# RobustFieldAutonomyLab/Distributional_RL_Navigation

Hardware: AMD Instinct MI355X
Metric: env steps/sec (whole node) at 65 536 envs; IQN grad-steps/sec (higher is better)
Workload: dtype f32; 1 GPU; 65536 envs/GPU + IQN training (act K=32, 8 quantiles, replay 100000, batch 256, 1 grad step(s) every 4 vector steps); envs_per_gpu=65536, n_cores=8, n_obstacles=10, precision=f64, learner=independent, ranks_per_gpu=1, act_variant=2, taus=per_env, resets=under_next_act, launches_per_grad_step=1, ablation=False

## Files before the change

distributional_rl_navigation_amd/csrc/mn_capi.hip:

```cpp
#include <math.h>
#include <stdio.h>
#include <stdlib.h>
#include <string.h>

#include <string>
#include <vector>

#include "mn_internal.h"
#include "mn_render_font.h"

struct mn_handle {
    MnArrays A;
    MnDev P;
    mn_params params;
    std::vector<void *> allocs;
    std::string err;
    int step_parity = 0;
    int last_parity = 0;
    uint32_t *seeds_dev = nullptr;
    uint32_t *mask_count = nullptr;
    int32_t *list_scratch = nullptr;
    double *peek_scratch = nullptr;
    double *obs64_buf = nullptr, *rew64_buf = nullptr;
    double *traj_trace = nullptr;
    int32_t traj_trace_steps = 0, traj_trace_sub = 0;
    int device = -1;
    std::vector<hipEvent_t> ev;
    int prof_max = 0, prof_n = 0;
    std::vector<hipEvent_t> ev_reset;
    int prof_reset_n = 0;
    hipStream_t side = nullptr;
    hipEvent_t ev_stepped = nullptr, ev_reset_end = nullptr;
    uint32_t *ready = nullptr;
    uint32_t tick = 0;
    bool reset_pending = false;
    volatile uint32_t *seen_host = nullptr;
    uint32_t *seen_dev = nullptr, *peak_dev = nullptr;
    int32_t under_act_max = MN_RESET_UNDER_ACT_MAX_DEFAULT;
// ... 140 lines not shown
    h->params = p;
    return MN_OK;
}

template <typename T>
static int dev_alloc(mn_handle *h, T **out, size_t count, bool zero = true) {
    void *p = nullptr;
    hipError_t e = hipMalloc(&p, count * sizeof(T));
    if (e != hipSuccess) { h->err = std::string("hipMalloc failed: ") + hipGetErrorString(e); return MN_ERR_ALLOC; }
    if (zero) { e = hipMemset(p, 0, count * sizeof(T)); if (e != hipSuccess) { h->err = hipGetErrorString(e); return MN_ERR_HIP; } }
    h->allocs.push_back(p);
    *out = (T *)p;
    return MN_OK;
}

extern "C" int mn_destroy(mn_handle *h) {
    if (!h) return MN_ERR_INVALID;
    int cur = -1;
    const bool moved = hipGetDevice(&cur) == hipSuccess && h->device >= 0 && cur != h->device;
    if (moved) (void)hipSetDevice(h->device);
    if (h->reset_owed) { const hipStream_t s = h->owed_stream; settle_owed(h, s); (void)hipStreamSynchronize(s); }
    for (hipEvent_t e : h->ev) (void)hipEventDestroy(e);
    for (hipEvent_t e : h->ev_reset) (void)hipEventDestroy(e);
    if (h->side) { (void)hipStreamSynchronize(h->side); (void)hipStreamDestroy(h->side); }
    if (h->ev_stepped) (void)hipEventDestroy(h->ev_stepped);
    if (h->ev_reset_end) (void)hipEventDestroy(h->ev_reset_end);
    if (h->seen_host) (void)hipHostFree((void *)h->seen_host);
    for (void *p : h->allocs) (void)hipFree(p);
    if (moved) (void)hipSetDevice(cur);
    delete h;
// ... 40 lines not shown
    {
        std::vector<double> v(np);
        for (size_t i = 0; i < np; ++i) v[i] = 5.0;
        (void)hipMemcpy(A.start_x, v.data(), np * 8, hipMemcpyHostToDevice);
        (void)hipMemcpy(A.start_y, v.data(), np * 8, hipMemcpyHostToDevice);
        for (size_t i = 0; i < np; ++i) v[i] = 45.0;
        (void)hipMemcpy(A.goal_x, v.data(), np * 8, hipMemcpyHostToDevice);
        (void)hipMemcpy(A.goal_y, v.data(), np * 8, hipMemcpyHostToDevice);
        std::vector<uint32_t> s(np);
        for (size_t i = 0; i < np; ++i) s[i] = (uint32_t)i;
        rc = mn_seed(h, s.data(), nullptr);
        if (rc) { g_create_err = h->err; mn_destroy(h); return rc; }
        hipError_t e = hipDeviceSynchronize();
        if (e != hipSuccess) { g_create_err = hipGetErrorString(e); mn_destroy(h); return MN_ERR_HIP; }
    }
    *out = h;
    return MN_OK;
}

extern "C" const char *mn_last_error(const mn_handle *h) { return h ? h->err.c_str() : g_create_err.c_str(); }
extern "C" int32_t mn_num_envs(const mn_handle *h) { return h ? h->A.n : 0; }

extern "C" int mn_set_params(mn_handle *h, const mn_params *p) {
    if (!h || !p) return MN_ERR_INVALID;
    if (p->precision != h->params.precision) return fail(h, MN_ERR_INVALID, "precision is fixed at mn_create");
    if (h->reset_owed) MN_ON_DEVICE(h);
    return derive(h, *p);
}

extern "C" int mn_get_params(const mn_handle *h, mn_params *p) {
// ... 395 lines not shown

extern "C" int mn_set_reset_owed_max_rows(mn_handle *h, int32_t owed_max_rows) {
    if (!h) return MN_ERR_INVALID;
    h->owed_max_rows = owed_max_rows;
    return MN_OK;
}

extern "C" int32_t mn_reset_is_owed(const mn_handle *h) { return h && h->reset_owed ? 1 : 0; }

bool mn_owed_reset_take(mn_handle *h, hipStream_t s, MnOwedReset *out) {
    if (!h || !h->reset_owed) return false;
    int cur = -1;
    if (hipGetDevice(&cur) != hipSuccess || cur != h->device) return false;
    if (s != h->owed_stream) (void)hipStreamSynchronize(h->owed_stream);
    const bool prof = h->prof_reset_n < h->prof_max;
    *out = MnOwedReset{&h->A, &h->P, h->params.precision, h->A.queue_count + h->last_parity * MN_QWORDS, h->A.queue, h->owed_obs, h->peak_dev, h->seen_dev,
                       mn_prep_reset_blocks(*h->seen_host, h->A.n), prof ? h->ev_reset[2 * h->prof_reset_n] : nullptr,
                       prof ? h->ev_reset[2 * h->prof_reset_n + 1] : nullptr};
    if (prof) h->prof_reset_n++;
    h->reset_owed = false;
    return true;
}
int mn_owed_reset_settle(mn_handle *h, hipStream_t s) {
    if (!h) return MN_OK;
    join_reset(h, s);
    return h->reset_owed ? fail(h, MN_ERR_INVALID, "the handle's owed reset lives on another HIP device") : MN_OK;
}

extern "C" int mn_set_reset_under_act_max(mn_handle *h, int32_t under_act_max, int64_t *last_seen) {
    if (!h) return MN_ERR_INVALID;
    h->under_act_max = under_act_max;
// ... 457 lines not shown
    int rc = range_ok(h, first, count);
    if (rc) return rc;
    if (count == 0) return MN_OK;
    if (!out) return MN_ERR_INVALID;
    if (!h->A.rew64) return fail(h, MN_ERR_INVALID, "float64 rewards are kept only with MN_PRECISION_F64 after mn_enable_obs64(h, 1)");
    MN_HIP(h, hipDeviceSynchronize());
    MN_HIP(h, hipMemcpy(out, h->A.rew64 + first, (size_t)count * 8, hipMemcpyDeviceToHost));
    return MN_OK;
}

extern "C" int mn_enable_obs64(mn_handle *h, int32_t on) {
    if (!h || on < 0 || on > 1) return MN_ERR_INVALID;
    MN_ON_DEVICE(h);
    if (h->params.precision != MN_PRECISION_F64) return fail(h, MN_ERR_INVALID, "float64 observation copies exist only with MN_PRECISION_F64");
    MN_HIP(h, hipDeviceSynchronize());
    if (!on) { h->A.obs64 = nullptr; h->A.rew64 = nullptr; return MN_OK; }
    if (!h->obs64_buf) {
        int rc = dev_alloc(h, &h->obs64_buf, (size_t)h->A.npad * MN_OBS_DIM);
        if (rc == MN_OK) rc = dev_alloc(h, &h->rew64_buf, (size_t)h->A.npad);
        if (rc) return rc;
    }
    h->A.obs64 = h->obs64_buf; h->A.rew64 = h->rew64_buf;
    return MN_OK;
}

extern "C" int mn_enable_trajectory(mn_handle *h, int32_t max_substeps) {
    if (!h || max_substeps < 1 || max_substeps > 1000) return MN_ERR_INVALID;
    MN_ON_DEVICE(h);
    if (h->params.precision != MN_PRECISION_F64) return fail(h, MN_ERR_INVALID, "sub-step trajectories are recorded only with MN_PRECISION_F64");
    if (h->A.traj && h->A.traj_n >= max_substeps) return MN_OK;
    MN_HIP(h, hipDeviceSynchronize());
    int rc = dev_alloc(h, &h->A.traj, (size_t)h->A.npad * max_substeps * 2);
    if (rc) return rc;
    h->A.traj_n = max_substeps;
    return MN_OK;
}

extern "C" int mn_get_trajectory(mn_handle *h, int32_t first, int32_t count, int32_t n_substeps, double *out) {
    int rc = range_ok(h, first, count);
    if (rc) return rc;
    if (count == 0) return MN_OK;
    if (!out || n_substeps < 1) return MN_ERR_INVALID;
    if (!h->A.traj || n_substeps > h->A.traj_n) return fail(h, MN_ERR_INVALID, "call mn_enable_trajectory(h, >= n_substeps) before stepping");
    MN_HIP(h, hipDeviceSynchronize());
    MN_HIP(h, hipMemcpy2D(out, (size_t)n_substeps * 16, h->A.traj + (size_t)first * h->A.traj_n * 2, (size_t)h->A.traj_n * 16,
                          (size_t)n_substeps * 16, count, hipMemcpyDeviceToHost));
    return MN_OK;
}

extern "C" int mn_peek_next_double(mn_handle *h, int32_t first, int32_t count, double *out) {
// ... 75 lines not shown
```

distributional_rl_navigation_amd/csrc/mn_internal.h:

```cpp
#pragma once
#include <hip/hip_runtime.h>
#include <stdint.h>

#include "marinenav_hip.h"

#define MN_WAVE 64
#define MN_PAD 256
#define MN_FIX_SCALE 16777216.0
#define MN_FIX_INV (1.0 / 16777216.0)
#define MN_TAB_ROWS (3 * MN_MAX_CORES + 3 * MN_MAX_OBS)

struct MnArrays {
    int32_t n, npad;
    double *x, *y, *theta, *speed, *vx, *vy;
    double *start_x, *start_y, *goal_x, *goal_y, *init_theta, *init_speed;
    int32_t *ep_t;
    int64_t *tot_t;
    int32_t *counts;
    double *cx, *cy, *cg;
    double *ox, *oy, *orad;
    int32_t *qcx, *qcy, *qox, *qoy;
    float *qcg, *qor;
    uint32_t *mt;
    int32_t *mt_pos;
// ... 99 lines not shown
int mn_iqn_rollout_image(mn_iqn_ctx *c, const float *const *weights, hipStream_t s, const uint32_t **image, uint32_t **words);
void mn_launch_dqn_pack(const float *const *weights, float *image_dev, hipStream_t s);
void mn_launch_rollout_dqn(const MnArrays &A, const MnDev &P, int precision, int n_steps, const float *image, float *obs_io, float *obs_trace,
                           float *reward_trace, uint8_t *done_trace, uint8_t *info_trace, int32_t *action_trace, float *q_trace, double *traj_trace, hipStream_t s);
void mn_launch_rollout_dqn_groups(const MnArrays &A, const MnDev &P, int precision, int n_steps, const float *images, int64_t image_stride, int n_groups,
                                  int rows_per_group, float *obs_io, float *obs_trace, float *reward_trace, uint8_t *done_trace, uint8_t *info_trace,
                                  int32_t *action_trace, float *q_trace, hipStream_t s);
void mn_launch_reset_under_act(const MnArrays &A, const MnDev &P, int precision, const uint32_t *count_dev, const int32_t *list_dev, float *obs,
                               uint32_t *ready, uint32_t tick, uint32_t *peak_dev, uint32_t *peak_host, hipStream_t s);
void mn_launch_reset(const MnArrays &A, const MnDev &P, int precision, const uint32_t *count_dev, uint32_t count_host,
                     const int32_t *list_dev, int mode, float *obs, hipStream_t s, uint32_t *peak_dev = nullptr, uint32_t *peak_host = nullptr, bool sharded = false);
#define MN_PREP_RESET_MIN_BLOCKS 256
#define MN_PREP_RESET_MAX_BLOCKS 8192
struct MnOwedReset {
    const MnArrays *A;
    const MnDev *P;
    int precision;
    const uint32_t *count_dev;
    const int32_t *list;
    float *obs;
    uint32_t *peak_dev, *peak_host;
    int blocks;
    hipEvent_t ev_begin, ev_end;
};
struct MnPrepLaunch {
    const float *const *weights;
    const float *consts;
    uint32_t *packed;
    bool pack;
    const uint64_t *rng_state;
// ... 33 lines not shown
```

distributional_rl_navigation_amd/csrc/mn_prep_reset.hip:

```cpp
#include <hip/hip_runtime.h>
#include <stdint.h>

#include "marinenav_hip.h"

#pragma clang fp contract(off)
#include "mn_reset_body.h"
#include "mn_done_queue.h"
#pragma clang fp contract(fast)

namespace {

#include "iqn_act_common.h"
#include "iqn_act_split.h"

constexpr int PR_PACK_BLOCKS = (sp::OFF_FB + MN_WAVE - 1) / MN_WAVE;

struct PrepArgs {
    IqnWeights w;
    const float *consts;
    uint32_t *packed;
    const uint64_t *rng_state;
    float *draws;
    int n;
    const float *cvar_row;
    float cvar;
    int pack_blocks;
    float eps;
    int32_t *actions;
    GreedyRows rows;
};

template <typename M, bool PARITY>
__global__ __launch_bounds__(MN_WAVE) void mn_prep_reset_kernel(MnArrays A, MnDev P, const uint32_t *__restrict__ count_dev, const int32_t *__restrict__ list,
                                                                float *__restrict__ obs_out, const MnSeen seen, int reset_blocks, PrepArgs a) {
    __shared__ MtLds S;
    __shared__ WorldLds W;
    if ((int)blockIdx.x < reset_blocks) {
        MnDoneQueue Q;
        const uint32_t count = Q.open(count_dev);
        mn_note_count(seen, count);
        for (uint32_t qi = blockIdx.x; qi < count; qi += (uint32_t)reset_blocks) mn_reset_env<M, PARITY>(A, P, S, W, Q.at(list, A.qcap, qi), 0, obs_out);
        return;
    }
    const int b = (int)blockIdx.x - reset_blocks;
    if (b < a.pack_blocks) {
        const int i = b * MN_WAVE + (int)threadIdx.x;
        if (i < sp::OFF_FB) a.packed[i] = sp::pack_word(a.w, a.consts, i);
        return;
    }
    if (a.rows.words) draw_block<true, MN_WAVE>(a.rng_state, a.draws, a.n, a.cvar_row, a.cvar, reset_blocks + a.pack_blocks, a.eps, a.actions, a.rows);
    else draw_block<false, MN_WAVE>(a.rng_state, a.draws, a.n, a.cvar_row, a.cvar, reset_blocks + a.pack_blocks);
}

}

int mn_prep_reset_blocks(uint32_t seen, int n) {
// ... 7 lines not shown
void mn_launch_prep_reset(const MnOwedReset &o, const MnPrepLaunch &p, hipStream_t s) {
    const MnSeen seen = {o.peak_dev, o.peak_host};
    PrepArgs a;
    const float *const *w = p.weights;
    a.w = {w[0], w[1], w[2], w[3], w[4], w[5], w[6], w[7], w[8], w[9], w[10], w[11], w[12], w[13]};
    a.consts = p.consts; a.packed = p.packed; a.rng_state = p.rng_state; a.draws = p.draws; a.n = p.n; a.cvar_row = p.cvar_row; a.cvar = p.cvar;
    a.pack_blocks = p.pack ? PR_PACK_BLOCKS : 0;
    a.eps = p.eps; a.actions = p.actions; a.rows = GreedyRows{p.rows_list, p.rows_words};
    const long items = ((long)p.n * (K_TAUS + 1) + 3) / 4;
    long draw = (items + MN_WAVE - 1) / MN_WAVE;
    if (draw > p.max_draw_blocks) draw = p.max_draw_blocks;
    if (draw < 1) draw = 1;
    const dim3 grid((unsigned)(o.blocks + a.pack_blocks + draw));
    if (o.ev_begin) (void)hipEventRecord(o.ev_begin, s);
    if (o.precision == MN_PRECISION_F64)
        hipLaunchKernelGGL((mn_prep_reset_kernel<double, true>), grid, dim3(MN_WAVE), 0, s, *o.A, *o.P, o.count_dev, o.list, o.obs, seen, o.blocks, a);
    else
        hipLaunchKernelGGL((mn_prep_reset_kernel<float, false>), grid, dim3(MN_WAVE), 0, s, *o.A, *o.P, o.count_dev, o.list, o.obs, seen, o.blocks, a);
    if (o.ev_end) (void)hipEventRecord(o.ev_end, s);
}
```

distributional_rl_navigation_amd/csrc/mn_reset.hip:

```cpp
#include "mn_reset_body.h"
#include "mn_done_queue.h"

#ifndef MN_RESET_MAX_BLOCKS
#define MN_RESET_MAX_BLOCKS 8192u
#endif

namespace {

template <typename M, bool PARITY>
__global__ __launch_bounds__(MN_WAVE) void mn_reset_kernel(MnArrays A, MnDev P, const uint32_t *__restrict__ count_dev,
                                                           uint32_t count_host, const int32_t *__restrict__ list, int mode,
                                                           float *__restrict__ obs_out, const MnSeen seen, int qcap) {
    __shared__ MtLds S;
    __shared__ WorldLds W;
    MnDoneQueue Q;
    const uint32_t count = qcap ? Q.open(count_dev) : (count_dev ? *count_dev : count_host);
    mn_note_count(seen, count);
    for (uint32_t qi = blockIdx.x; qi < count; qi += gridDim.x)
        mn_reset_env<M, PARITY>(A, P, S, W, qcap ? Q.at(list, qcap, qi) : (list ? list[qi] : (int)qi), mode, obs_out);
}

template <typename M, bool PARITY>
__global__ __launch_bounds__(MN_WAVE, 5) void mn_reset_under_act_kernel(MnArrays A, MnDev P, const uint32_t *__restrict__ count_dev,
                                                                        const int32_t *__restrict__ list, float *__restrict__ obs_out,
                                                                        uint32_t *__restrict__ ready, uint32_t tick, const MnSeen seen) {
    __shared__ MtCarryLds S;
    __shared__ WorldLds W;
    MnDoneQueue Q;
    const uint32_t count = Q.open(count_dev);
    mn_note_count(seen, count);
    for (uint32_t qi = blockIdx.x; qi < count; qi += gridDim.x)
        mn_reset_env<M, PARITY, MtInPlace>(A, P, S, W, Q.at(list, A.qcap, qi), 0, obs_out, ready, tick);
}

// ... 71 lines not shown
    while (__builtin_amdgcn_s_memrealtime() - t0 < 100ull * us) __builtin_amdgcn_s_sleep(64);
}
void mn_launch_sleep(uint32_t us, hipStream_t s) { hipLaunchKernelGGL(mn_sleep_kernel, dim3(1), dim3(MN_WAVE), 0, s, us); }

void mn_launch_seed(const MnArrays &A, const uint32_t *seeds_dev, hipStream_t s) {
    hipLaunchKernelGGL(mn_seed_kernel, dim3((A.n + 255) / 256), dim3(256), 0, s, A, seeds_dev);
}

void mn_launch_mask_to_queue(const MnArrays &A, const uint8_t *mask, uint32_t *count, int32_t *list, hipStream_t s) {
    hipLaunchKernelGGL(mn_mask_to_queue_kernel, dim3((A.n + 255) / 256), dim3(256), 0, s, A, mask, count, list);
}

void mn_launch_peek(const MnArrays &A, int first, int count, double *out_dev, hipStream_t s) {
    hipLaunchKernelGGL(mn_peek_kernel, dim3((count + 255) / 256), dim3(256), 0, s, A, first, count, out_dev);
}
```

distributional_rl_navigation_amd/csrc/mn_reset_body.h:

```cpp
#pragma once
#include "mn_device.h"

#ifdef MN_ABLATION
#define MN_RSKIP(bit) ((P.debug_skip & (bit)) != 0)
#else
#define MN_RSKIP(bit) false
#endif

#define MT_N 624
#define MT_M 397

__device__ __forceinline__ uint32_t mt_temper(uint32_t y) {
    y ^= (y >> 11);
    y ^= (y << 7) & 0x9d2c5680u;
    y ^= (y << 15) & 0xefc60000u;
    y ^= (y >> 18);
    return y;
}

__device__ __forceinline__ uint32_t mt_twist(uint32_t cur, uint32_t nxt, uint32_t far) {
    const uint32_t y = (cur & 0x80000000u) | (nxt & 0x7fffffffu);
    return far ^ (y >> 1) ^ ((y & 1u) ? 0x9908b0dfu : 0u);
}

struct MtLds {
    uint32_t key[MT_N];
    uint32_t carry[8];
};

__device__ __forceinline__ void mt_regenerate(MtLds &S, int lane) {
    for (int base = 0; base < MT_N - 1; base += MN_WAVE) {
        const int i = base + lane;
        uint32_t v = 0;
        const bool ok = i < MT_N - 1;
        if (ok) {
            const int j = i + MT_M < MT_N ? i + MT_M : i + MT_M - MT_N;
            v = mt_twist(S.key[i], S.key[i + 1], S.key[j]);
        }
        __syncthreads();
        if (ok) S.key[i] = v;
        __syncthreads();
    }
    if (lane == 0) S.key[MT_N - 1] = mt_twist(S.key[MT_N - 1], S.key[0], S.key[MT_M - 1]);
    __syncthreads();
}

struct MtCursor {
    int pos;
    int carry_n;
    bool regen;
};

__device__ __forceinline__ int mt_ensure(MtLds &S, MtCursor &c, int w, int lane) {
    int avail = c.carry_n + (MT_N - c.pos);
    if (avail < w) {
        const int rem = MT_N - c.pos;
        if (lane < rem) S.carry[c.carry_n + lane] = mt_temper(S.key[c.pos + lane]);
        __syncthreads();
        c.carry_n += rem;
        mt_regenerate(S, lane);
// ... 9 lines not shown
    return j < c.carry_n ? S.carry[j] : mt_temper(S.key[c.pos + j - c.carry_n]);
}

__device__ __forceinline__ double mt_double_at(const MtLds &S, const MtCursor &c, int j) {
    const uint32_t a = mt_word(S, c, j) >> 5, b = mt_word(S, c, j + 1) >> 6;
    return (a * 67108864.0 + b) / 9007199254740992.0;
}

__device__ __forceinline__ void mt_advance(MtCursor &c, int words) {
    c.pos += words - c.carry_n;
    c.carry_n = 0;
}

struct MtInLds {
    using Shared = MtLds;
    MtLds &S;
    MtCursor c;
    __device__ __forceinline__ MtInLds(MtLds &s) : S(s) {}
    __device__ __forceinline__ void load(const MnArrays &A, int e, int lane) {
        for (int j = lane; j < MT_N; j += MN_WAVE) S.key[j] = A.mt[(size_t)e * MT_N + j];
        c.pos = A.mt_pos[e];
        c.carry_n = 0;
        c.regen = false;
        __syncthreads();
    }
    __device__ __forceinline__ int ensure(int w, int lane) { return mt_ensure(S, c, w, lane); }
    template <int N>
    __device__ __forceinline__ void fetch(int j, double (&d)[N]) const {
#pragma unroll
        for (int q = 0; q < N; ++q) d[q] = mt_double_at(S, c, j + 2 * q);
    }
    __device__ __forceinline__ void advance(int words) { mt_advance(c, words); }
    __device__ __forceinline__ void store(const MnArrays &A, int e, int lane, bool skip) {
        if (c.regen && !skip) for (int j = lane; j < MT_N; j += MN_WAVE) A.mt[(size_t)e * MT_N + j] = S.key[j];
    }
};

struct MtCarryLds { uint32_t carry[8]; };
struct MtInPlace {
    using Shared = MtCarryLds;
    MtCarryLds &S;
    uint32_t *k;
    MtCursor c;
    __device__ __forceinline__ MtInPlace(MtCarryLds &s) : S(s), k(nullptr) {}
    static __device__ __forceinline__ uint32_t ld(const uint32_t *p) { return __hip_atomic_load(p, __ATOMIC_RELAXED, __HIP_MEMORY_SCOPE_AGENT); }
    static __device__ __forceinline__ void st(uint32_t *p, uint32_t v) { __hip_atomic_store(p, v, __ATOMIC_RELAXED, __HIP_MEMORY_SCOPE_AGENT); }
    __device__ __forceinline__ void load(const MnArrays &A, int e, int lane) {
        k = A.mt + (size_t)e * MT_N;
        c.pos = A.mt_pos[e];
        c.carry_n = 0;
        c.regen = false;
    }
    __device__ __forceinline__ void regenerate(int lane) {
        uint32_t a[4], b[4], u[4], v[4], f[4];
#pragma unroll
// ... 131 lines not shown
        if (d2 > t2 * (1.0 + 1.0e-11)) return true;
    } else {
        const double tr = 2 * P.core_r, tr2 = tr * tr;
        if (d2 < tr2 * (1.0 - 1.0e-11)) return true;
        if (d2 > tr2 * (1.0 + 1.0e-11)) {
            const double Gl = Gi > Gj ? Gi : Gj, Gs = Gi < Gj ? Gi : Gj;
            const double a = P.p * Gs, b = Gl * P.core_r + tr * a;
            const double lhs = a * a * d2, rhs = b * b;
            if (lhs < rhs * (1.0 - 1.0e-11)) return false;
            if (lhs > rhs * (1.0 + 1.0e-11)) return true;
        }
    }
    return cores_compatible_exact(P, sqrt(d2), gi, gj);
}

template <typename M, bool PARITY, typename RNG = MtInLds>
__device__ __forceinline__ void mn_reset_env(const MnArrays &A, const MnDev &P, typename RNG::Shared &S, WorldLds &W, int e, int mode,
                                             float *__restrict__ obs_out, uint32_t *__restrict__ ready = nullptr, uint32_t tick = 0u) {
    const int lane = threadIdx.x & (MN_WAVE - 1);
    const int np = A.npad;
    __syncthreads();
    int nc = 0, no = 0;
    double sx, sy, gx, gy, th0, sp0;

    if (mode == 0) {
        int want_c = P.num_cores, want_o = P.num_obs;
        double min_dis = P.min_start_goal_dis;
        if (P.n_stages > 0) {
            const int64_t tt = (int64_t)((double)A.tot_t[e] * P.timestep_scale);
            int cntle = 0;
            for (int i = 0; i < P.n_stages; ++i) cntle += (P.sched_t[i] - tt <= 0) ? 1 : 0;
            int idx = cntle - 1;
            if (idx < 0) idx += P.n_stages;
            want_c = P.sched_nc[idx]; want_o = P.sched_no[idx]; min_dis = P.sched_md[idx];
        }
        want_c = want_c > MN_MAX_CORES ? MN_MAX_CORES : want_c;
        want_o = want_o > MN_MAX_OBS ? MN_MAX_OBS : want_o;

        RNG rng(S);
        rng.load(A, e, lane);

        sx = A.start_x[e]; sy = A.start_y[e]; gx = A.goal_x[e]; gy = A.goal_y[e];
        if (P.reset_start_and_goal && !MN_RSKIP(32)) {
            int tried = 0;
            double best = 0.0;
            for (;;) {
                int nb = rng.ensure(8, lane);
                nb = nb < 500 - tried ? nb : 500 - tried;
                const bool mine = lane < nb;
                double s0 = 0, s1 = 0, g0 = 0, g1 = 0, d = -1.0;
                if (mine) {
                    double u[4];
                    rng.template fetch<4>(8 * lane, u);
                    s0 = P.sg_lo_x + P.sg_span_x * u[0];
                    s1 = P.sg_lo_y + P.sg_span_y * u[1];
                    g0 = P.sg_lo_x + P.sg_span_x * u[2];
                    g1 = P.sg_lo_y + P.sg_span_y * u[3];
// ... 13 lines not shown
                        if (od > bm || (od == bm && ol < bl)) { bm = od; bl = ol; }
                    }
                    pick = bm > best ? bl : -1;
                    used = nb; finished = (tried + nb) >= 500;
                }
                if (pick >= 0) {
                    best = bcast(d, pick);
                    sx = bcast(s0, pick); sy = bcast(s1, pick); gx = bcast(g0, pick); gy = bcast(g1, pick);
                }
                tried += used;
                rng.advance(8 * used);
                if (finished) break;
            }
        }

        if (want_c > 0 && !MN_RSKIP(64)) {
            int tried = 0;
            for (;;) {
                int nb = rng.ensure(8, lane);
                nb = nb < 500 - tried ? nb : 500 - tried;
                const bool mine = lane < nb;
                double x = 0, y = 0, g = 1.0;
                bool valid = false;
                if (mine) {
                    double u[4];
                    rng.template fetch<4>(8 * lane, u);
                    x = 0.0 + P.c_span_x * u[0];
                    y = 0.0 + P.c_span_y * u[1];
                    const bool clockwise = u[2] > P.binom_q;
                    const double v_edge = P.v_lo + P.v_span * u[3];
                    const double Gamma = P.two_pi_r * v_edge;
// ... 10 lines not shown
                    if (!m) break;
                    const int j = first_lane(m);
                    const double xj = bcast(x, j), yj = bcast(y, j), gj = bcast(g, j);
                    if (lane == j) { W.cx[nc] = x; W.cy[nc] = y; W.cg[nc] = g; valid = false; }
                    else if (valid && lane > j) valid = cores_compatible(P, xj, yj, gj, x, y, g);
                    ++nc;
                    if (nc == want_c) { used = j + 1; break; }
                }
                __syncthreads();
                tried += used;
                rng.advance(8 * used);
                if (nc == want_c || tried >= 500) break;
            }
        }

        if (want_o > 0 && !MN_RSKIP(128)) {
            int tried = 0;
            for (;;) {
                int nb = rng.ensure(6, lane);
                nb = nb < 500 - tried ? nb : 500 - tried;
                const bool mine = lane < nb;
                double x = 0, y = 0, r = 0;
                bool valid = false;
                if (mine) {
                    double u[3];
                    rng.template fetch<3>(6 * lane, u);
                    x = P.o_lo + P.o_span_x * u[0];
                    y = P.o_lo + P.o_span_y * u[1];
                    r = P.or_lo + P.or_span * u[2];
                    valid = !(x - r < 0.0 || x + r > P.width) && !(y - r < 0.0 || y + r > P.height) &&
                            !dist_lt((x - sx) * (x - sx) + (y - sy) * (y - sy), r + P.clear_r) &&
// ... 16 lines not shown
                    if (lane == j) { W.ox[no] = x; W.oy[no] = y; W.orad[no] = r; valid = false; }
                    else if (valid && lane > j) {
                        const double dx = xj - x, dy = yj - y;
                        valid = !dist_le(dx * dx + dy * dy, rj + r);
                    }
                    ++no;
                    if (no == want_o) { used = j + 1; break; }
                }
                __syncthreads();
                tried += used;
                rng.advance(6 * used);
                if (no == want_o || tried >= 500) break;
            }
        }

        if (P.random_reset_state) {
            rng.ensure(4, lane);
            double u[2];
            rng.template fetch<2>(0, u);
            th0 = 0.0 + (P.two_pi - 0.0) * u[0];
            sp0 = 0.0 + (P.max_speed - 0.0) * u[1];
            rng.advance(4);
        } else {
            th0 = P.init_theta; sp0 = P.init_speed;
        }

        __syncthreads();
        rng.store(A, e, lane, MN_RSKIP(512));
        if (lane < MN_MAX_CORES) {
            const bool v = lane < nc;
            A.cx[lane * np + e] = v ? W.cx[lane] : 0.0;
            A.cy[lane * np + e] = v ? W.cy[lane] : 0.0;
            A.cg[lane * np + e] = v ? W.cg[lane] : 0.0;
        }
        if (lane < MN_MAX_OBS) {
            const bool v = lane < no;
            A.ox[lane * np + e] = v ? W.ox[lane] : 0.0;
            A.oy[lane * np + e] = v ? W.oy[lane] : 0.0;
            A.orad[lane * np + e] = v ? W.orad[lane] : 0.0;
        }
        if (lane == 0) {
            A.mt_pos[e] = rng.c.pos;
            A.counts[e] = nc | (no << 8);
            A.start_x[e] = sx; A.start_y[e] = sy; A.goal_x[e] = gx; A.goal_y[e] = gy;
            A.init_theta[e] = th0; A.init_speed[e] = sp0;
        }
    } else {
        const int cnt = A.counts[e];
        nc = cnt & 0xff; no = (cnt >> 8) & 0xff;
        if (lane < nc) { W.cx[lane] = A.cx[lane * np + e]; W.cy[lane] = A.cy[lane * np + e]; W.cg[lane] = A.cg[lane * np + e]; }
        if (lane < no) { W.ox[lane] = A.ox[lane * np + e]; W.oy[lane] = A.oy[lane * np + e]; W.orad[lane] = A.orad[lane * np + e]; }
        sx = A.start_x[e]; sy = A.start_y[e]; gx = A.goal_x[e]; gy = A.goal_y[e];
        th0 = A.init_theta[e]; sp0 = A.init_speed[e];
    }
    __syncthreads();

    if (lane < MN_MAX_CORES) {
        const bool v = lane < nc;
        A.qcx[lane * np + e] = v ? __double2int_rn(W.cx[lane] * MN_FIX_SCALE) : 0;
        A.qcy[lane * np + e] = v ? __double2int_rn(W.cy[lane] * MN_FIX_SCALE) : 0;
        A.qcg[lane * np + e] = v ? (float)W.cg[lane] : 0.0f;
    }
    if (lane < MN_MAX_OBS) {
        const bool v = lane < no;
        A.qox[lane * np + e] = v ? __double2int_rn(W.ox[lane] * MN_FIX_SCALE) : 0;
        A.qoy[lane * np + e] = v ? __double2int_rn(W.oy[lane] * MN_FIX_SCALE) : 0;
        A.qor[lane * np + e] = v ? (float)W.orad[lane] : 0.0f;
    }

    double cvx = 0.0, cvy = 0.0;
    {
        const double i1 = P.inv_two_pi_r2, i2 = P.inv_two_pi;
        for (int k = 0; k < nc; ++k) {
            double ux, uy;
            mn_core_velocity<double, true>(W.cx[k] - sx, W.cy[k] - sy, W.cg[k], i1, i2, ux, uy);
            cvx += ux; cvy += uy;
        }
    }
    double sn, cs;
    sincos(th0, &sn, &cs);
    const double velx = sp0 * cs + cvx, vely = sp0 * sn + cvy;

    if (lane < MN_NUM_BEAMS) {
        const double angle = th0 + P.beam_rel[lane];
        const bool up = fabs(angle - 0.5 * 3.141592653589793) < 1e-03;
        const bool down = fabs(angle - 3 * 3.141592653589793 / 2) < 1e-03;
        double bx = P.beam_cos[lane], by = P.beam_sin[lane];
        if (up || down) {
            const double sg = up ? 1.0 : -1.0;
            bx = sg * sn; by = sg * cs;
        }
        MnBeam<M> beam;
        beam.init();
        for (int k = 0; k < (MN_RSKIP(256) ? 0 : no); ++k) {
            const double mx = W.ox[k] - sx, my = W.oy[k] - sy;
            double tc, h2;
            mn_beam_geom(cs * mx + sn * my, -sn * mx + cs * my, W.orad[k] * W.orad[k], bx, by, tc, h2);
            beam.update(tc, h2, (M)P.sonar_range);
        }
        const double td = PARITY ? (double)beam.dist : beam.dist64();
        W.beam[lane][0] = beam.hit() ? td * bx : 0.0;
        W.beam[lane][1] = beam.hit() ? td * by : 0.0;
    }
    __syncthreads();
    if (lane < MN_OBS_DIM) {
        double v;
        const double gdx = gx - sx, gdy = gy - sy;
        if (lane == 0) v = cs * velx + sn * vely;
        else if (lane == 1) v = -sn * velx + cs * vely;
        else if (lane == 2) v = cs * gdx + sn * gdy;
        else if (lane == 3) v = -sn * gdx + cs * gdy;
        else v = W.beam[(lane - 4) >> 1][(lane - 4) & 1];
        if (obs_out) {
            if (ready) __hip_atomic_store(reinterpret_cast<uint32_t *>(obs_out) + (size_t)e * MN_OBS_DIM + lane, __float_as_uint((float)v), __ATOMIC_RELAXED, __HIP_MEMORY_SCOPE_AGENT);
            else obs_out[(size_t)e * MN_OBS_DIM + lane] = (float)v;
        }
        if (PARITY && A.obs64) A.obs64[(size_t)e * MN_OBS_DIM + lane] = v;
    }
    if (lane == 0) {
        A.x[e] = sx; A.y[e] = sy; A.theta[e] = th0; A.speed[e] = sp0;
        A.vx[e] = velx; A.vy[e] = vely;
        A.ep_t[e] = 0;
    }
    if (ready) {
        asm volatile("s_waitcnt vmcnt(0)" ::: "memory");
        if (lane == 0) __hip_atomic_store(ready + e, tick, __ATOMIC_RELAXED, __HIP_MEMORY_SCOPE_AGENT);
    }
}
```

Baseline: 1.016 billion env steps/s.

## Rework env reset: precomputed MT doubles, wave-parallel rejection sampling, scalar-memory tail stores

Reset kernels now hold the Mersenne Twister state as precomputed doubles in shared memory (MtDoubles), with raw words kept in registers and written back only after a regeneration. Obstacle and core placement use wave-parallel rejection sampling with cheap distance tests, falling back to exact comparisons only when a lane is inside a tolerance band. Core velocities are computed one per lane and then reduced. Tail stores read array pointers through a device copy of MnArrays via scalar loads to reduce kernel-argument register pressure, and optional s_memtime phase instrumentation is added. Together these aim to cut reset latency but add complexity and carry exactness risk in the banded comparisons.

```diff
diff --git a/distributional_rl_navigation_amd/csrc/mn_capi.hip b/distributional_rl_navigation_amd/csrc/mn_capi.hip
--- a/distributional_rl_navigation_amd/csrc/mn_capi.hip
+++ b/distributional_rl_navigation_amd/csrc/mn_capi.hip
@@ -22,6 +22,7 @@
     int32_t *list_scratch = nullptr;
     double *peek_scratch = nullptr;
     double *obs64_buf = nullptr, *rew64_buf = nullptr;
+    MnArrays *A_mem = nullptr;
     double *traj_trace = nullptr;
     int32_t traj_trace_steps = 0, traj_trace_sub = 0;
     int device = -1;
@@ -192,6 +193,15 @@
     return MN_OK;
 }
 
+static int sync_arrays(mn_handle *h) {
+    if (!h->A_mem) {
+        const int rc = dev_alloc(h, &h->A_mem, 1, false);
+        if (rc) return rc;
+    }
+    MN_HIP(h, hipMemcpy(h->A_mem, &h->A, sizeof(MnArrays), hipMemcpyHostToDevice));
+    return MN_OK;
+}
+
 extern "C" int mn_destroy(mn_handle *h) {
     if (!h) return MN_ERR_INVALID;
     int cur = -1;
@@ -262,6 +272,7 @@
         hipError_t e = hipDeviceSynchronize();
         if (e != hipSuccess) { g_create_err = hipGetErrorString(e); mn_destroy(h); return MN_ERR_HIP; }
     }
+    if ((rc = sync_arrays(h)) != MN_OK) { g_create_err = h->err; mn_destroy(h); return rc; }
     *out = h;
     return MN_OK;
 }
@@ -687,7 +698,7 @@
     if (hipGetDevice(&cur) != hipSuccess || cur != h->device) return false;
     if (s != h->owed_stream) (void)hipStreamSynchronize(h->owed_stream);
     const bool prof = h->prof_reset_n < h->prof_max;
-    *out = MnOwedReset{&h->A, &h->P, h->params.precision, h->A.queue_count + h->last_parity * MN_QWORDS, h->A.queue, h->owed_obs, h->peak_dev, h->seen_dev,
+    *out = MnOwedReset{&h->A, h->A_mem, &h->P, h->params.precision, h->A.queue_count + h->last_parity * MN_QWORDS, h->A.queue, h->owed_obs, h->peak_dev, h->seen_dev,
                        mn_prep_reset_blocks(*h->seen_host, h->A.n), prof ? h->ev_reset[2 * h->prof_reset_n] : nullptr,
                        prof ? h->ev_reset[2 * h->prof_reset_n + 1] : nullptr};
     if (prof) h->prof_reset_n++;
@@ -1175,14 +1186,14 @@
     MN_ON_DEVICE(h);
     if (h->params.precision != MN_PRECISION_F64) return fail(h, MN_ERR_INVALID, "float64 observation copies exist only with MN_PRECISION_F64");
     MN_HIP(h, hipDeviceSynchronize());
-    if (!on) { h->A.obs64 = nullptr; h->A.rew64 = nullptr; return MN_OK; }
+    if (!on) { h->A.obs64 = nullptr; h->A.rew64 = nullptr; return sync_arrays(h); }
     if (!h->obs64_buf) {
         int rc = dev_alloc(h, &h->obs64_buf, (size_t)h->A.npad * MN_OBS_DIM);
         if (rc == MN_OK) rc = dev_alloc(h, &h->rew64_buf, (size_t)h->A.npad);
         if (rc) return rc;
     }
     h->A.obs64 = h->obs64_buf; h->A.rew64 = h->rew64_buf;
-    return MN_OK;
+    return sync_arrays(h);
 }
 
 extern "C" int mn_enable_trajectory(mn_handle *h, int32_t max_substeps) {
@@ -1194,7 +1205,7 @@
     int rc = dev_alloc(h, &h->A.traj, (size_t)h->A.npad * max_substeps * 2);
     if (rc) return rc;
     h->A.traj_n = max_substeps;
-    return MN_OK;
+    return sync_arrays(h);
 }
 
 extern "C" int mn_get_trajectory(mn_handle *h, int32_t first, int32_t count, int32_t n_substeps, double *out) {
diff --git a/distributional_rl_navigation_amd/csrc/mn_internal.h b/distributional_rl_navigation_amd/csrc/mn_internal.h
--- a/distributional_rl_navigation_amd/csrc/mn_internal.h
+++ b/distributional_rl_navigation_amd/csrc/mn_internal.h
@@ -137,6 +137,7 @@
 #define MN_PREP_RESET_MAX_BLOCKS 8192
 struct MnOwedReset {
     const MnArrays *A;
+    const MnArrays *A_mem;
     const MnDev *P;
     int precision;
     const uint32_t *count_dev;
diff --git a/distributional_rl_navigation_amd/csrc/mn_prep_reset.hip b/distributional_rl_navigation_amd/csrc/mn_prep_reset.hip
--- a/distributional_rl_navigation_amd/csrc/mn_prep_reset.hip
+++ b/distributional_rl_navigation_amd/csrc/mn_prep_reset.hip
@@ -32,14 +32,14 @@
 
 template <typename M, bool PARITY>
 __global__ __launch_bounds__(MN_WAVE) void mn_prep_reset_kernel(MnArrays A, MnDev P, const uint32_t *__restrict__ count_dev, const int32_t *__restrict__ list,
-                                                                float *__restrict__ obs_out, const MnSeen seen, int reset_blocks, PrepArgs a) {
-    __shared__ MtLds S;
+                                                                float *__restrict__ obs_out, const MnSeen seen, int reset_blocks, const MnArrays *A_mem, PrepArgs a) {
+    __shared__ MtDblLds S;
     __shared__ WorldLds W;
     if ((int)blockIdx.x < reset_blocks) {
         MnDoneQueue Q;
         const uint32_t count = Q.open(count_dev);
         mn_note_count(seen, count);
-        for (uint32_t qi = blockIdx.x; qi < count; qi += (uint32_t)reset_blocks) mn_reset_env<M, PARITY>(A, P, S, W, Q.at(list, A.qcap, qi), 0, obs_out);
+        for (uint32_t qi = blockIdx.x; qi < count; qi += (uint32_t)reset_blocks) mn_reset_env<M, PARITY, MtDoubles, true, true>(A, P, S, W, Q.at(list, A.qcap, qi), 0, obs_out, nullptr, 0u, A_mem);
         return;
     }
     const int b = (int)blockIdx.x - reset_blocks;
@@ -77,8 +77,8 @@
     const dim3 grid((unsigned)(o.blocks + a.pack_blocks + draw));
     if (o.ev_begin) (void)hipEventRecord(o.ev_begin, s);
     if (o.precision == MN_PRECISION_F64)
-        hipLaunchKernelGGL((mn_prep_reset_kernel<double, true>), grid, dim3(MN_WAVE), 0, s, *o.A, *o.P, o.count_dev, o.list, o.obs, seen, o.blocks, a);
+        hipLaunchKernelGGL((mn_prep_reset_kernel<double, true>), grid, dim3(MN_WAVE), 0, s, *o.A, *o.P, o.count_dev, o.list, o.obs, seen, o.blocks, o.A_mem, a);
     else
-        hipLaunchKernelGGL((mn_prep_reset_kernel<float, false>), grid, dim3(MN_WAVE), 0, s, *o.A, *o.P, o.count_dev, o.list, o.obs, seen, o.blocks, a);
+        hipLaunchKernelGGL((mn_prep_reset_kernel<float, false>), grid, dim3(MN_WAVE), 0, s, *o.A, *o.P, o.count_dev, o.list, o.obs, seen, o.blocks, o.A_mem, a);
     if (o.ev_end) (void)hipEventRecord(o.ev_end, s);
 }
diff --git a/distributional_rl_navigation_amd/csrc/mn_reset.hip b/distributional_rl_navigation_amd/csrc/mn_reset.hip
--- a/distributional_rl_navigation_amd/csrc/mn_reset.hip
+++ b/distributional_rl_navigation_amd/csrc/mn_reset.hip
@@ -1,3 +1,7 @@
+#ifdef MN_ABLATION
+__device__ unsigned long long g_reset_phase[8];
+#define MN_RESET_PHASE_VAR g_reset_phase
+#endif
 #include "mn_reset_body.h"
 #include "mn_done_queue.h"
 
@@ -11,13 +15,13 @@
 __global__ __launch_bounds__(MN_WAVE) void mn_reset_kernel(MnArrays A, MnDev P, const uint32_t *__restrict__ count_dev,
                                                            uint32_t count_host, const int32_t *__restrict__ list, int mode,
                                                            float *__restrict__ obs_out, const MnSeen seen, int qcap) {
-    __shared__ MtLds S;
+    __shared__ MtDblLds S;
     __shared__ WorldLds W;
     MnDoneQueue Q;
     const uint32_t count = qcap ? Q.open(count_dev) : (count_dev ? *count_dev : count_host);
     mn_note_count(seen, count);
     for (uint32_t qi = blockIdx.x; qi < count; qi += gridDim.x)
-        mn_reset_env<M, PARITY>(A, P, S, W, qcap ? Q.at(list, qcap, qi) : (list ? list[qi] : (int)qi), mode, obs_out);
+        mn_reset_env<M, PARITY, MtDoubles>(A, P, S, W, qcap ? Q.at(list, qcap, qi) : (list ? list[qi] : (int)qi), mode, obs_out);
 }
 
 template <typename M, bool PARITY>
@@ -119,3 +123,14 @@
 void mn_launch_peek(const MnArrays &A, int first, int count, double *out_dev, hipStream_t s) {
     hipLaunchKernelGGL(mn_peek_kernel, dim3((count + 255) / 256), dim3(256), 0, s, A, first, count, out_dev);
 }
+
+#ifdef MN_ABLATION
+extern "C" int mn_debug_reset_phases(unsigned long long *out_host, int reset) {
+    if (hipMemcpyFromSymbol(out_host, HIP_SYMBOL(g_reset_phase), sizeof(unsigned long long) * 8) != hipSuccess) return MN_ERR_HIP;
+    if (reset) {
+        const unsigned long long z[8] = {0};
+        if (hipMemcpyToSymbol(HIP_SYMBOL(g_reset_phase), z, sizeof(z)) != hipSuccess) return MN_ERR_HIP;
+    }
+    return MN_OK;
+}
+#endif
diff --git a/distributional_rl_navigation_amd/csrc/mn_reset_body.h b/distributional_rl_navigation_amd/csrc/mn_reset_body.h
--- a/distributional_rl_navigation_amd/csrc/mn_reset_body.h
+++ b/distributional_rl_navigation_amd/csrc/mn_reset_body.h
@@ -5,6 +5,18 @@
 #define MN_RSKIP(bit) ((P.debug_skip & (bit)) != 0)
 #else
 #define MN_RSKIP(bit) false
+#endif
+#if defined(MN_ABLATION) && defined(MN_RESET_PHASE_VAR)
+#define MN_RTICK_BEGIN() unsigned long long mn_rtick[7] = {0, 0, 0, 0, 0, 0, 0}; __builtin_amdgcn_sched_barrier(0); \
+        unsigned long long mn_rtick_prev = __builtin_amdgcn_s_memtime(); __builtin_amdgcn_sched_barrier(0)
+#define MN_RTICK(k) do { __builtin_amdgcn_sched_barrier(0); const unsigned long long t_ = __builtin_amdgcn_s_memtime(); \
+        mn_rtick[k] = t_ - mn_rtick_prev; mn_rtick_prev = t_; __builtin_amdgcn_sched_barrier(0); } while (0)
+#define MN_RTICK_END() do { if (blockIdx.x == 0 && threadIdx.x == 0) { for (int k_ = 0; k_ < 7; ++k_) atomicAdd(&MN_RESET_PHASE_VAR[k_], mn_rtick[k_]); \
+        atomicAdd(&MN_RESET_PHASE_VAR[7], 1ull); } } while (0)
+#else
+#define MN_RTICK_BEGIN() do { } while (0)
+#define MN_RTICK(k) do { } while (0)
+#define MN_RTICK_END() do { } while (0)
 #endif
 
 #define MT_N 624
@@ -28,22 +40,23 @@
     uint32_t carry[8];
 };
 
-__device__ __forceinline__ void mt_regenerate(MtLds &S, int lane) {
+__device__ __forceinline__ void mt_regenerate_words(uint32_t *key, int lane) {
     for (int base = 0; base < MT_N - 1; base += MN_WAVE) {
         const int i = base + lane;
         uint32_t v = 0;
         const bool ok = i < MT_N - 1;
         if (ok) {
             const int j = i + MT_M < MT_N ? i + MT_M : i + MT_M - MT_N;
-            v = mt_twist(S.key[i], S.key[i + 1], S.key[j]);
+            v = mt_twist(key[i], key[i + 1], key[j]);
         }
         __syncthreads();
-        if (ok) S.key[i] = v;
+        if (ok) key[i] = v;
         __syncthreads();
     }
-    if (lane == 0) S.key[MT_N - 1] = mt_twist(S.key[MT_N - 1], S.key[0], S.key[MT_M - 1]);
+    if (lane == 0) key[MT_N - 1] = mt_twist(key[MT_N - 1], key[0], key[MT_M - 1]);
     __syncthreads();
 }
+__device__ __forceinline__ void mt_regenerate(MtLds &S, int lane) { mt_regenerate_words(S.key, lane); }
 
 struct MtCursor {
     int pos;
@@ -83,6 +96,7 @@
 
 struct MtInLds {
     using Shared = MtLds;
+    static constexpr bool SHORT_CHAIN = true;
     MtLds &S;
     MtCursor c;
     __device__ __forceinline__ MtInLds(MtLds &s) : S(s) {}
@@ -105,9 +119,96 @@
     }
 };
 
+union MtDblLds {
+    double v[4 + MT_N / 2];
+    struct { uint32_t pad[8]; uint32_t key[MT_N]; } raw;
+};
+__device__ __forceinline__ double mt_double_of(uint32_t w0, uint32_t w1) {
+    const uint32_t a = mt_temper(w0) >> 5, b = mt_temper(w1) >> 6;
+    return (a * 67108864.0 + b) / 9007199254740992.0;
+}
+struct MtDoubles {
+    using Shared = MtDblLds;
+    static constexpr bool SHORT_CHAIN = true;
+    static constexpr int PAIRS = MT_N / 2, PER_LANE = (MT_N / 2 + MN_WAVE - 1) / MN_WAVE;
+    MtDblLds &S;
+    MtCursor c;
+    uint2 raw[PER_LANE];
+    __device__ __forceinline__ MtDoubles(MtDblLds &s) : S(s) {}
+    __device__ __forceinline__ void form(int first, int lane) {
+#pragma unroll
+        for (int k = 0; k < PER_LANE; ++k) {
+            const int q = lane + MN_WAVE * k;
+            if (MN_WAVE * k + MN_WAVE > first && q < PAIRS) S.v[4 + q] = mt_double_of(raw[k].x, raw[k].y);
+        }
+    }
+    __device__ __forceinline__ void load(const MnArrays &A, int e, int lane) {
+        const uint2 *row = reinterpret_cast<const uint2 *>(A.mt + (size_t)e * MT_N);
+#pragma unroll
+        for (int k = 0; k < PER_LANE; ++k) {
+            const int q = lane + MN_WAVE * k;
+            raw[k] = q < PAIRS ? row[q] : make_uint2(0u, 0u);
+        }
+        c.pos = A.mt_pos[e];
+        c.carry_n = 0;
+        c.regen = false;
+        form(c.pos >> 1, lane);
+        __syncthreads();
+    }
+    __device__ __forceinline__ int ensure(int w, int lane) {
+        int avail = c.carry_n + (MT_N - c.pos);
+        if (avail < w) {
+            const int rem = MT_N - c.pos, nd = rem >> 1;
+            double keep = 0.0;
+            if (lane < nd) keep = S.v[4 + (c.pos >> 1) + lane];
+            __syncthreads();
+            if (lane < nd) S.v[4 - nd + lane] = keep;
+#pragma unroll
+            for (int k = 0; k < PER_LANE; ++k) {
+                const int q = lane + MN_WAVE * k;
+                if (q < PAIRS) { S.raw.key[2 * q] = raw[k].x; S.raw.key[2 * q + 1] = raw[k].y; }
+            }
+            __syncthreads();
+            mt_regenerate_words(S.raw.key, lane);
+#pragma unroll
+            for (int k = 0; k < PER_LANE; ++k) {
+                const int q = lane + MN_WAVE * k;
+                if (q < PAIRS) raw[k] = make_uint2(S.raw.key[2 * q], S.raw.key[2 * q + 1]);
+            }
+            __syncthreads();
+            form(0, lane);
+            __syncthreads();
+            c.carry_n = rem;
+            c.regen = true;
+            c.pos = 0;
+            avail = c.carry_n + MT_N;
+        }
+        const int n = avail / w;
+        return n < MN_WAVE ? n : MN_WAVE;
+    }
+    template <int N>
+    __device__ __forceinline__ void fetch(int j, double (&d)[N]) const {
+        const int at = 4 + ((c.pos - c.carry_n + j) >> 1);
+#pragma unroll
+        for (int q = 0; q < N; ++q) d[q] = S.v[at + q];
+    }
+    __device__ __forceinline__ void advance(int words) { mt_advance(c, words); }
+    __device__ __forceinline__ void store(const MnArrays &A, int e, int lane, bool skip) {
+        if (c.regen && !skip) {
+            uint2 *row = reinterpret_cast<uint2 *>(A.mt + (size_t)e * MT_N);
+#pragma unroll
+            for (int k = 0; k < PER_LANE; ++k) {
+                const int q = lane + MN_WAVE * k;
+                if (q < PAIRS) row[q] = raw[k];
+            }
+        }
+    }
+};
+
 struct MtCarryLds { uint32_t carry[8]; };
 struct MtInPlace {
     using Shared = MtCarryLds;
+    static constexpr bool SHORT_CHAIN = false;
     MtCarryLds &S;
     uint32_t *k;
     MtCursor c;
@@ -269,12 +370,46 @@
     return cores_compatible_exact(P, sqrt(d2), gi, gj);
 }
 
-template <typename M, bool PARITY, typename RNG = MtInLds>
+#ifndef MN_REAL_BRANCH
+#define MN_REAL_BRANCH() asm volatile("" ::: "memory")
+#endif
+__device__ __forceinline__ bool dist_lt_sel(double d2, double T, bool &band) {
+    const double t2 = T * T;
+    const bool lt = d2 < t2 * (1.0 - MN_BAND), gt = d2 > t2 * (1.0 + MN_BAND);
+    band = !(lt | gt);
+    return lt;
+}
+__device__ __forceinline__ bool dist_le_sel(double d2, double T, bool &band) { return dist_lt_sel(d2, T, band); }
+
+__device__ __forceinline__ bool cores_compatible_sel(const MnDev &P, double xi, double yi, double gi, double xj, double yj, double gj, bool &band) {
+    const double dx = xi - xj, dy = yi - yj;
+    const double d2 = dx * dx + dy * dy;
+    const double Gi = fabs(gi), Gj = fabs(gj);
+    const double T = (Gi + Gj) * P.inv_two_pi_vrel, t2 = T * T;
+    const bool s_no = d2 < t2 * (1.0 - 1.0e-11), s_yes = d2 > t2 * (1.0 + 1.0e-11);
+    const double tr = 2 * P.core_r, tr2 = tr * tr;
+    const bool o_in = d2 < tr2 * (1.0 - 1.0e-11), o_out = d2 > tr2 * (1.0 + 1.0e-11);
+    const double Gl = Gi > Gj ? Gi : Gj, Gs = Gi < Gj ? Gi : Gj;
+    const double a = P.p * Gs, b = Gl * P.core_r + tr * a;
+    const double lhs = a * a * d2, rhs = b * b;
+    const bool l_no = lhs < rhs * (1.0 - 1.0e-11), l_yes = lhs > rhs * (1.0 + 1.0e-11);
+    const bool same = (gi > 0.0) == (gj > 0.0);
+    const bool s_dec = s_no | s_yes, o_dec = o_in | (o_out & (l_no | l_yes)), o_val = o_in | (o_out & l_yes);
+    band = !((same & s_dec) | (!same & o_dec));
+    return (same & s_yes) | (!same & o_val);
+}
+
+typedef const __attribute__((address_space(4))) MnArrays *MnArraysMem;
+#define MN_TAIL(f) (TAIL_MEM ? at->f : A.f)
+template <typename M, bool PARITY, typename RNG = MtInLds, bool SHORT = RNG::SHORT_CHAIN, bool TAIL_MEM = false>
 __device__ __forceinline__ void mn_reset_env(const MnArrays &A, const MnDev &P, typename RNG::Shared &S, WorldLds &W, int e, int mode,
-                                             float *__restrict__ obs_out, uint32_t *__restrict__ ready = nullptr, uint32_t tick = 0u) {
+                                             float *__restrict__ obs_out, uint32_t *__restrict__ ready = nullptr, uint32_t tick = 0u,
+                                             const MnArrays *A_mem = nullptr) {
     const int lane = threadIdx.x & (MN_WAVE - 1);
     const int np = A.npad;
+    MnArraysMem at = nullptr;
     __syncthreads();
+    MN_RTICK_BEGIN();
     int nc = 0, no = 0;
     double sx, sy, gx, gy, th0, sp0;
 
@@ -292,10 +427,12 @@
         want_c = want_c > MN_MAX_CORES ? MN_MAX_CORES : want_c;
         want_o = want_o > MN_MAX_OBS ? MN_MAX_OBS : want_o;
 
+        if (SHORT) { sx = A.start_x[e]; sy = A.start_y[e]; gx = A.goal_x[e]; gy = A.goal_y[e]; }
         RNG rng(S);
         rng.load(A, e, lane);
-
-        sx = A.start_x[e]; sy = A.start_y[e]; gx = A.goal_x[e]; gy = A.goal_y[e];
+        MN_RTICK(0);
+
+        if (!SHORT) { sx = A.start_x[e]; sy = A.start_y[e]; gx = A.goal_x[e]; gy = A.goal_y[e]; }
         if (P.reset_start_and_goal && !MN_RSKIP(32)) {
             int tried = 0;
             double best = 0.0;
@@ -339,7 +476,67 @@
             }
         }
 
-        if (want_c > 0 && !MN_RSKIP(64)) {
+        MN_RTICK(1);
+
+        double acx = 0.0, acy = 0.0, acg = 0.0;
+        if (SHORT && want_c > 0 && !MN_RSKIP(64)) {
+            int tried = 0;
+            for (;;) {
+                int nb = rng.ensure(8, lane);
+                nb = nb < 500 - tried ? nb : 500 - tried;
+                const bool mine = lane < nb;
+                double u[4] = {0.0, 0.0, 0.0, 0.0};
+                if (mine) rng.template fetch<4>(8 * lane, u);
+                const double x = 0.0 + P.c_span_x * u[0];
+                const double y = 0.0 + P.c_span_y * u[1];
+                const bool clockwise = u[2] > P.binom_q;
+                const double v_edge = P.v_lo + P.v_span * u[3];
+                const double Gamma = P.two_pi_r * v_edge;
+                const double g = clockwise ? Gamma : -Gamma;
+                const double ds2 = (x - sx) * (x - sx) + (y - sy) * (y - sy), dg2 = (x - gx) * (x - gx) + (y - gy) * (y - gy);
+                const bool inside = !(x - P.core_r < 0.0 || x + P.core_r > P.width) && !(y - P.core_r < 0.0 || y + P.core_r > P.width) ;
+                bool b0, b1;
+                bool near_s = dist_lt_sel(ds2, P.core_r + P.clear_r, b0), near_g = dist_lt_sel(dg2, P.core_r + P.clear_r, b1);
+                if (__any(mine & (b0 | b1))) {
+                    MN_REAL_BRANCH();
+                    near_s = dist_lt(ds2, P.core_r + P.clear_r); near_g = dist_lt(dg2, P.core_r + P.clear_r);
+                }
+                bool valid = mine & inside & !near_s & !near_g;
+                for (int i = 0; i < nc; ++i) {
+                    const double xi = bcast(acx, i), yi = bcast(acy, i), gi = bcast(acg, i);
+                    bool bi;
+                    bool ok = cores_compatible_sel(P, xi, yi, gi, x, y, g, bi);
+                    if (__any(valid & bi)) {
+                        MN_REAL_BRANCH();
+                        ok = cores_compatible(P, xi, yi, gi, x, y, g);
+                    }
+                    valid = valid & ok;
+                }
+                int used = nb;
+                for (;;) {
+                    const unsigned long long m = __ballot(valid);
+                    if (!m) break;
+                    const int j = first_lane(m);
+                    const double xj = bcast(x, j), yj = bcast(y, j), gj = bcast(g, j);
+                    if (lane == nc) { acx = xj; acy = yj; acg = gj; }
+                    bool bj;
+                    bool ok = cores_compatible_sel(P, xj, yj, gj, x, y, g, bj);
+                    if (__any(valid & (lane > j) & bj)) {
+                        MN_REAL_BRANCH();
+                        ok = cores_compatible(P, xj, yj, gj, x, y, g);
+                    }
+                    valid = valid & (lane > j) & ok;
+                    ++nc;
+                    if (nc == want_c) { used = j + 1; break; }
+                }
+                tried += used;
+                rng.advance(8 * used);
+                if (nc == want_c || tried >= 500) break;
+            }
+            if (lane < nc) { W.cx[lane] = acx; W.cy[lane] = acy; W.cg[lane] = acg; }
+            __syncthreads();
+        }
+        if (!SHORT && want_c > 0 && !MN_RSKIP(64)) {
             int tried = 0;
             for (;;) {
                 int nb = rng.ensure(8, lane);
@@ -380,7 +577,75 @@
             }
         }
 
-        if (want_o > 0 && !MN_RSKIP(128)) {
+        MN_RTICK(2);
+
+        if (SHORT && want_o > 0 && !MN_RSKIP(128)) {
+            double aox = 0.0, aoy = 0.0, aor = 0.0;
+            int tried = 0;
+            for (;;) {
+                int nb = rng.ensure(6, lane);
+                nb = nb < 500 - tried ? nb : 500 - tried;
+                const bool mine = lane < nb;
+                double u[3] = {0.0, 0.0, 0.0};
+                if (mine) rng.template fetch<3>(6 * lane, u);
+                const double x = P.o_lo + P.o_span_x * u[0];
+                const double y = P.o_lo + P.o_span_y * u[1];
+                const double r = P.or_lo + P.or_span * u[2];
+                const double ds2 = (x - sx) * (x - sx) + (y - sy) * (y - sy), dg2 = (x - gx) * (x - gx) + (y - gy) * (y - gy);
+                const bool inside = !(x - r < 0.0 || x + r > P.width) && !(y - r < 0.0 || y + r > P.height);
+                bool b0, b1;
+                bool near_s = dist_lt_sel(ds2, r + P.clear_r, b0), near_g = dist_lt_sel(dg2, r + P.clear_r, b1);
+                if (__any(mine & (b0 | b1))) {
+                    MN_REAL_BRANCH();
+                    near_s = dist_lt(ds2, r + P.clear_r); near_g = dist_lt(dg2, r + P.clear_r);
+                }
+                bool valid = mine & inside & !near_s & !near_g;
+                for (int i = 0; i < nc; ++i) {
+                    const double dx = bcast(acx, i) - x, dy = bcast(acy, i) - y;
+                    bool bi;
+                    bool hit = dist_le_sel(dx * dx + dy * dy, P.core_r + r, bi);
+                    if (__any(valid & bi)) {
+                        MN_REAL_BRANCH();
+                        hit = dist_le(dx * dx + dy * dy, P.core_r + r);
+                    }
+                    valid = valid & !hit;
+                }
+                for (int i = 0; i < no; ++i) {
+                    const double dx = bcast(aox, i) - x, dy = bcast(aoy, i) - y, T = bcast(aor, i) + r;
+                    bool bi;
+                    bool hit = dist_le_sel(dx * dx + dy * dy, T, bi);
+                    if (__any(valid & bi)) {
+                        MN_REAL_BRANCH();
+                        hit = dist_le(dx * dx + dy * dy, T);
+                    }
+                    valid = valid & !hit;
+                }
+                int used = nb;
+                for (;;) {
+                    const unsigned long long m = __ballot(valid);
+                    if (!m) break;
+                    const int j = first_lane(m);
+                    const double xj = bcast(x, j), yj = bcast(y, j), rj = bcast(r, j);
+                    if (lane == no) { aox = xj; aoy = yj; aor = rj; }
+                    const double dx = xj - x, dy = yj - y;
+                    bool bj;
+                    bool hit = dist_le_sel(dx * dx + dy * dy, rj + r, bj);
+                    if (__any(valid & (lane > j) & bj)) {
+                        MN_REAL_BRANCH();
+                        hit = dist_le(dx * dx + dy * dy, rj + r);
+                    }
+                    valid = valid & (lane > j) & !hit;
+                    ++no;
+                    if (no == want_o) { used = j + 1; break; }
+                }
+                tried += used;
+                rng.advance(6 * used);
+                if (no == want_o || tried >= 500) break;
+            }
+            if (lane < no) { W.ox[lane] = aox; W.oy[lane] = aoy; W.orad[lane] = aor; }
+            __syncthreads();
+        }
+        if (!SHORT && want_o > 0 && !MN_RSKIP(128)) {
             int tried = 0;
             for (;;) {
                 int nb = rng.ensure(6, lane);
@@ -427,6 +692,8 @@
             }
         }
 
+        MN_RTICK(3);
+
         if (P.random_reset_state) {
             rng.ensure(4, lane);
             double u[2];
@@ -439,25 +706,34 @@
         }
 
         __syncthreads();
+        if (TAIL_MEM) {
+            unsigned long long u = (unsigned long long)A_mem;
+            asm volatile("" : "+s"(u));
+            at = (MnArraysMem)u;
+            asm volatile("" ::"s"(at->cx), "s"(at->cy), "s"(at->cg), "s"(at->ox), "s"(at->oy), "s"(at->orad), "s"(at->qcx), "s"(at->qcy), "s"(at->qcg), "s"(at->qox),
+                         "s"(at->qoy), "s"(at->qor), "s"(at->mt_pos), "s"(at->counts), "s"(at->start_x), "s"(at->start_y), "s"(at->goal_x), "s"(at->goal_y),
+                         "s"(at->init_theta), "s"(at->init_speed));
+        }
         rng.store(A, e, lane, MN_RSKIP(512));
         if (lane < MN_MAX_CORES) {
             const bool v = lane < nc;
-            A.cx[lane * np + e] = v ? W.cx[lane] : 0.0;
-            A.cy[lane * np + e] = v ? W.cy[lane] : 0.0;
-            A.cg[lane * np + e] = v ? W.cg[lane] : 0.0;
+            MN_TAIL(cx)[lane * np + e] = v ? W.cx[lane] : 0.0;
+            MN_TAIL(cy)[lane * np + e] = v ? W.cy[lane] : 0.0;
+            MN_TAIL(cg)[lane * np + e] = v ? W.cg[lane] : 0.0;
         }
         if (lane < MN_MAX_OBS) {
             const bool v = lane < no;
-            A.ox[lane * np + e] = v ? W.ox[lane] : 0.0;
-            A.oy[lane * np + e] = v ? W.oy[lane] : 0.0;
-            A.orad[lane * np + e] = v ? W.orad[lane] : 0.0;
+            MN_TAIL(ox)[lane * np + e] = v ? W.ox[lane] : 0.0;
+            MN_TAIL(oy)[lane * np + e] = v ? W.oy[lane] : 0.0;
+            MN_TAIL(orad)[lane * np + e] = v ? W.orad[lane] : 0.0;
         }
         if (lane == 0) {
-            A.mt_pos[e] = rng.c.pos;
-            A.counts[e] = nc | (no << 8);
-            A.start_x[e] = sx; A.start_y[e] = sy; A.goal_x[e] = gx; A.goal_y[e] = gy;
-            A.init_theta[e] = th0; A.init_speed[e] = sp0;
-        }
+            MN_TAIL(mt_pos)[e] = rng.c.pos;
+            MN_TAIL(counts)[e] = nc | (no << 8);
+            MN_TAIL(start_x)[e] = sx; MN_TAIL(start_y)[e] = sy; MN_TAIL(goal_x)[e] = gx; MN_TAIL(goal_y)[e] = gy;
+            MN_TAIL(init_theta)[e] = th0; MN_TAIL(init_speed)[e] = sp0;
+        }
+        MN_RTICK(4);
     } else {
         const int cnt = A.counts[e];
         nc = cnt & 0xff; no = (cnt >> 8) & 0xff;
@@ -470,21 +746,27 @@
 
     if (lane < MN_MAX_CORES) {
         const bool v = lane < nc;
-        A.qcx[lane * np + e] = v ? __double2int_rn(W.cx[lane] * MN_FIX_SCALE) : 0;
-        A.qcy[lane * np + e] = v ? __double2int_rn(W.cy[lane] * MN_FIX_SCALE) : 0;
-        A.qcg[lane * np + e] = v ? (float)W.cg[lane] : 0.0f;
+        MN_TAIL(qcx)[lane * np + e] = v ? __double2int_rn(W.cx[lane] * MN_FIX_SCALE) : 0;
+        MN_TAIL(qcy)[lane * np + e] = v ? __double2int_rn(W.cy[lane] * MN_FIX_SCALE) : 0;
+        MN_TAIL(qcg)[lane * np + e] = v ? (float)W.cg[lane] : 0.0f;
     }
     if (lane < MN_MAX_OBS) {
         const bool v = lane < no;
-        A.qox[lane * np + e] = v ? __double2int_rn(W.ox[lane] * MN_FIX_SCALE) : 0;
-        A.qoy[lane * np + e] = v ? __double2int_rn(W.oy[lane] * MN_FIX_SCALE) : 0;
-        A.qor[lane * np + e] = v ? (float)W.orad[lane] : 0.0f;
+        MN_TAIL(qox)[lane * np + e] = v ? __double2int_rn(W.ox[lane] * MN_FIX_SCALE) : 0;
+        MN_TAIL(qoy)[lane * np + e] = v ? __double2int_rn(W.oy[lane] * MN_FIX_SCALE) : 0;
+        MN_TAIL(qor)[lane * np + e] = v ? (float)W.orad[lane] : 0.0f;
     }
 
     double cvx = 0.0, cvy = 0.0;
     {
         const double i1 = P.inv_two_pi_r2, i2 = P.inv_two_pi;
-        for (int k = 0; k < nc; ++k) {
+        if (SHORT) {
+            double ux = 0.0, uy = 0.0;
+            const int kk = lane < nc ? lane : 0;
+            mn_core_velocity<double, true>(W.cx[kk] - sx, W.cy[kk] - sy, W.cg[kk], i1, i2, ux, uy);
+            for (int k = 0; k < nc; ++k) { cvx += bcast(ux, k); cvy += bcast(uy, k); }
+        }
+        for (int k = 0; k < (SHORT ? 0 : nc); ++k) {
             double ux, uy;
             mn_core_velocity<double, true>(W.cx[k] - sx, W.cy[k] - sy, W.cg[k], i1, i2, ux, uy);
             cvx += ux; cvy += uy;
@@ -493,6 +775,7 @@
     double sn, cs;
     sincos(th0, &sn, &cs);
     const double velx = sp0 * cs + cvx, vely = sp0 * sn + cvy;
+    MN_RTICK(5);
 
     if (lane < MN_NUM_BEAMS) {
         const double angle = th0 + P.beam_rel[lane];
@@ -516,6 +799,7 @@
         W.beam[lane][1] = beam.hit() ? td * by : 0.0;
     }
     __syncthreads();
+    if (TAIL_MEM && mode == 0) asm volatile("" ::"s"(at->x), "s"(at->y), "s"(at->theta), "s"(at->speed), "s"(at->vx), "s"(at->vy), "s"(at->ep_t), "s"(at->obs64));
     if (lane < MN_OBS_DIM) {
         double v;
         const double gdx = gx - sx, gdy = gy - sy;
@@ -528,15 +812,17 @@
             if (ready) __hip_atomic_store(reinterpret_cast<uint32_t *>(obs_out) + (size_t)e * MN_OBS_DIM + lane, __float_as_uint((float)v), __ATOMIC_RELAXED, __HIP_MEMORY_SCOPE_AGENT);
             else obs_out[(size_t)e * MN_OBS_DIM + lane] = (float)v;
         }
-        if (PARITY && A.obs64) A.obs64[(size_t)e * MN_OBS_DIM + lane] = v;
+        if (PARITY && MN_TAIL(obs64)) MN_TAIL(obs64)[(size_t)e * MN_OBS_DIM + lane] = v;
     }
     if (lane == 0) {
-        A.x[e] = sx; A.y[e] = sy; A.theta[e] = th0; A.speed[e] = sp0;
-        A.vx[e] = velx; A.vy[e] = vely;
-        A.ep_t[e] = 0;
+        MN_TAIL(x)[e] = sx; MN_TAIL(y)[e] = sy; MN_TAIL(theta)[e] = th0; MN_TAIL(speed)[e] = sp0;
+        MN_TAIL(vx)[e] = velx; MN_TAIL(vy)[e] = vely;
+        MN_TAIL(ep_t)[e] = 0;
     }
     if (ready) {
         asm volatile("s_waitcnt vmcnt(0)" ::: "memory");
         if (lane == 0) __hip_atomic_store(ready + e, tick, __ATOMIC_RELAXED, __HIP_MEMORY_SCOPE_AGENT);
     }
-}
+    MN_RTICK(6);
+    MN_RTICK_END();
+}
```

Result: faster. 1.138 billion env steps/s (median of 6 runs) (+12.1%).
